# alshai/rowbowt

Measured on AMD Instinct MI355X. Metric: reads/s (100 bp, count+locate), higher is better.
Workload: dtype u32/u64

## Files before the change

rowbowt_amd/csrc/rbg_runs_device.hpp:

```cpp
#pragma once

#include "rbg_device.hpp"

namespace rbg {
namespace {



constexpr uint32_t kStageCap = 256u;
constexpr uint32_t kStageWords = kStageCap / 16u + 1u;
constexpr uint32_t kStageWaveBytes = kStageWords * 64u * 4u;
typedef __attribute__((address_space(3))) uint32_t lds_u32;

struct StageTab { uint32_t code_lo, code_hi, byte_lo, byte_hi, shift; };
__device__ __forceinline__ uint32_t stage_chunk(const u32x4 w, const StageTab &T, uint32_t (&diff)[4]) {
    const uint32_t x[4] = {w.x, w.y, w.z, w.w};
    uint32_t c8[4];
#pragma unroll
    for (int t = 0; t < 4; ++t) {
        const uint32_t idx = (x[t] >> T.shift) & 0x07070707u;
        const uint32_t code = __builtin_amdgcn_perm(T.code_hi, T.code_lo, idx);
        diff[t] = x[t] ^ __builtin_amdgcn_perm(T.byte_hi, T.byte_lo, idx);
        c8[t] = (code * 0x40100401u) >> 24;
    }
    return c8[3] | (c8[2] << 8) | (c8[1] << 16) | (c8[0] << 24);
}
__device__ __forceinline__ uint32_t nibble_bytes(const uint32_t nib) { return (((nib & 15u) * 0x00204081u) & 0x01010101u) * 0xFFu; }
__device__ __forceinline__ bool stage_read(const uint4 *__restrict__ chunks16, const uint64_t beg, const uint64_t end, const StageTab &T, lds_u32 *col, uint32_t &chunks_out) {
    chunks_out = 0;
    if (end <= beg) return false;
    uint64_t ci = (end - 1) >> 4;
    const uint64_t ci_lo = beg >> 4;
    const uint32_t hi_b = static_cast<uint32_t>(end - 1) & 15u, lo_b = static_cast<uint32_t>(beg) & 15u;
    const uint32_t skip2 = 2u * (15u - hi_b);
    uint32_t nwords = static_cast<uint32_t>((end - beg + 15) >> 4);
    uint32_t bad = 0;
    uint32_t d[4];
    u32x4 w = as_global<u32x4>(static_cast<const void *>(chunks16))[ci];
    uint32_t prev = stage_chunk(w, T, d);
    {
        uint32_t vm = (2u << hi_b) - 1u;
        if (ci == ci_lo) vm &= ~((1u << lo_b) - 1u);
        bad |= (d[0] & nibble_bytes(vm)) | (d[1] & nibble_bytes(vm >> 4)) | (d[2] & nibble_bytes(vm >> 8)) | (d[3] & nibble_bytes(vm >> 12));
    }
    chunks_out = static_cast<uint32_t>(ci - ci_lo) + 1u;
    while (nwords) {
        uint32_t next = 0;
        if (ci > ci_lo) {
            --ci;
            w = as_global<u32x4>(static_cast<const void *>(chunks16))[ci];
            next = stage_chunk(w, T, d);
            if (ci == ci_lo) {
                const uint32_t vm = ~((1u << lo_b) - 1u);
                bad |= (d[0] & nibble_bytes(vm)) | (d[1] & nibble_bytes(vm >> 4)) | (d[2] & nibble_bytes(vm >> 8)) | (d[3] & nibble_bytes(vm >> 12));
            } else {
                bad |= d[0] | d[1] | d[2] | d[3];
            }
        }
        *col = __builtin_amdgcn_alignbit(next, prev, skip2);
        col += 64;
        prev = next;
        --nwords;
    }
    return bad != 0;
}

__device__ __forceinline__ uint32_t staged_bits(const lds_u32 *col, const uint32_t t, const uint32_t nsym) {
    const lds_u32 *cw = col + (t >> 4) * 64u;
    const uint32_t v = __builtin_amdgcn_alignbit(cw[64], cw[0], (t & 15u) * 2u);
    return nsym >= 16u ? v : (v & ((1u << (2u * nsym)) - 1u));
}

__device__ __forceinline__ uint32_t run_record(const uint32_t *s_tab_first, uint32_t adv, uint32_t acc) { return s_tab_first[adv - 1] + acc; }

struct RunStep {
    uint64_t F = 0, c_before = 0, c_upto = 0;
    bool inside = false;
    uint64_t samp_e = 0;
};


}
}
```

Before: 2.419 billion.

## Batch chunk loads in stage_read to overlap global memory latency

Restructures the staging loop so each lane issues up to G (default 8) 16-byte global loads back to back, separated by a scheduling barrier, before processing them. The old loop had one dependent load per iteration. The loop now runs until no lane in the wave has chunks left, using a ballot. The byte-packing in stage_chunk also swaps shifts and ORs for two perm instructions. The batching raises register pressure and issues redundant clamped loads for lanes with few chunks. It also drops the early return for empty ranges and changes the edge logic for the final word.

```diff
diff --git a/rowbowt_amd/csrc/rbg_runs_device.hpp b/rowbowt_amd/csrc/rbg_runs_device.hpp
--- a/rowbowt_amd/csrc/rbg_runs_device.hpp
+++ b/rowbowt_amd/csrc/rbg_runs_device.hpp
@@ -21,46 +21,47 @@
         const uint32_t idx = (x[t] >> T.shift) & 0x07070707u;
         const uint32_t code = __builtin_amdgcn_perm(T.code_hi, T.code_lo, idx);
         diff[t] = x[t] ^ __builtin_amdgcn_perm(T.byte_hi, T.byte_lo, idx);
-        c8[t] = (code * 0x40100401u) >> 24;
+        c8[t] = code * 0x40100401u;
     }
-    return c8[3] | (c8[2] << 8) | (c8[1] << 16) | (c8[0] << 24);
+    return __builtin_amdgcn_perm(c8[2], c8[3], 0x0c0c0703u) | __builtin_amdgcn_perm(c8[0], c8[1], 0x07030c0cu);
 }
 __device__ __forceinline__ uint32_t nibble_bytes(const uint32_t nib) { return (((nib & 15u) * 0x00204081u) & 0x01010101u) * 0xFFu; }
+template <int G = 8>
 __device__ __forceinline__ bool stage_read(const uint4 *__restrict__ chunks16, const uint64_t beg, const uint64_t end, const StageTab &T, lds_u32 *col, uint32_t &chunks_out) {
-    chunks_out = 0;
-    if (end <= beg) return false;
-    uint64_t ci = (end - 1) >> 4;
-    const uint64_t ci_lo = beg >> 4;
+    const uint64_t ci_top = (end - 1) >> 4, ci_lo = beg >> 4;
     const uint32_t hi_b = static_cast<uint32_t>(end - 1) & 15u, lo_b = static_cast<uint32_t>(beg) & 15u;
     const uint32_t skip2 = 2u * (15u - hi_b);
-    uint32_t nwords = static_cast<uint32_t>((end - beg + 15) >> 4);
-    uint32_t bad = 0;
-    uint32_t d[4];
-    u32x4 w = as_global<u32x4>(static_cast<const void *>(chunks16))[ci];
-    uint32_t prev = stage_chunk(w, T, d);
-    {
-        uint32_t vm = (2u << hi_b) - 1u;
-        if (ci == ci_lo) vm &= ~((1u << lo_b) - 1u);
-        bad |= (d[0] & nibble_bytes(vm)) | (d[1] & nibble_bytes(vm >> 4)) | (d[2] & nibble_bytes(vm >> 8)) | (d[3] & nibble_bytes(vm >> 12));
-    }
-    chunks_out = static_cast<uint32_t>(ci - ci_lo) + 1u;
-    while (nwords) {
-        uint32_t next = 0;
-        if (ci > ci_lo) {
-            --ci;
-            w = as_global<u32x4>(static_cast<const void *>(chunks16))[ci];
-            next = stage_chunk(w, T, d);
-            if (ci == ci_lo) {
-                const uint32_t vm = ~((1u << lo_b) - 1u);
-                bad |= (d[0] & nibble_bytes(vm)) | (d[1] & nibble_bytes(vm >> 4)) | (d[2] & nibble_bytes(vm >> 8)) | (d[3] & nibble_bytes(vm >> 12));
-            } else {
-                bad |= d[0] | d[1] | d[2] | d[3];
+    const uint32_t nwords = static_cast<uint32_t>((end - beg + 15) >> 4);
+    const uint32_t nch = end > beg ? static_cast<uint32_t>(ci_top - ci_lo) + 1u : 0u;
+    const auto *gtop = as_global<u32x4>(static_cast<const void *>(chunks16)) + ci_top;
+    int32_t rem = static_cast<int32_t>(nch) - 1;
+    bool first = true;
+    uint32_t bad = 0, prev = 0;
+    chunks_out = nch;
+    for (; __ballot(rem >= 0) != 0; rem -= G, gtop -= G, col += 64 * G, first = false) {
+        if (rem < 0) continue;
+        u32x4 w[G];
+#pragma unroll
+        for (int s = 0; s < G; ++s) w[s] = *(gtop - (s < rem ? s : rem));
+        __builtin_amdgcn_sched_barrier(0);
+#pragma unroll
+        for (int s = 0; s < G; ++s) {
+            if (s == 0 || s <= rem) {
+                const bool is_top = s == 0 && first, is_bottom = s == rem;
+                uint32_t d[4];
+                const uint32_t cur = stage_chunk(w[s], T, d);
+                if (is_top || is_bottom) {
+                    uint32_t vm = is_top ? (2u << hi_b) - 1u : ~0u;
+                    if (is_bottom) vm &= ~((1u << lo_b) - 1u);
+                    bad |= (d[0] & nibble_bytes(vm)) | (d[1] & nibble_bytes(vm >> 4)) | (d[2] & nibble_bytes(vm >> 8)) | (d[3] & nibble_bytes(vm >> 12));
+                } else {
+                    bad |= d[0] | d[1] | d[2] | d[3];
+                }
+                if (!is_top) col[64 * (s - 1)] = __builtin_amdgcn_alignbit(cur, prev, skip2);
+                if (is_bottom && nwords == nch) col[64 * s] = __builtin_amdgcn_alignbit(0u, cur, skip2);
+                prev = cur;
             }
         }
-        *col = __builtin_amdgcn_alignbit(next, prev, skip2);
-        col += 64;
-        prev = next;
-        --nwords;
     }
     return bad != 0;
 }
```

Result: no change. 2.399 billion (-0.8%).
